# pairlab/leibnizgym

Measured on AMD Instinct MI355X. Metric: env-steps/sec (whole node), trifinger_difficulty_4 @65536 envs, 1/2/4/8 GPUs, higher is better.
Workload: dtype f32

## Files before the change

### leibnizgym_amd/csrc/tf_roles.h

```cpp
#pragma once
#include <type_traits>

#include "tf_contact.h"

#define NT 256

enum { M_ACT_IN = 1, M_RESETS = 2, M_TORQUE = 4, M_SIM = 8, M_POST = 16, M_FINISH = 32, M_ACT_RAND = 64  };
#define M_FUSED_STEP (M_ACT_IN | M_RESETS | M_TORQUE | M_SIM | M_POST | M_FINISH)
#define M_FUSED_STEP_RAND (M_FUSED_STEP | M_ACT_RAND)
#define M_FUSED_RESET (M_RESETS | M_TORQUE | M_SIM | M_POST)

#define L_REC(f) (30 * (f))
#define R_A 0
#define R_DIR 6
#define R_RXD 15
#define R_U 24
#define R_DL 27
#define P_AW 0
#define P_BW 3
#define P_MINV 6
#define P_S1 12
#define P_C1 13
#define P_P2 14
#define P_P3 17
#define P_VQ 20
#define L_POSE_A 23
#define L_POSE_B 53
#define L_WALL 90
#define L_PARK(f) L_REC(f)
#define PK_FC 0
#define PK_LINK 4
#define PK_TF 5
#define PK_TW 8
#define PK_TAU 11
#define PK_FT 14
#define L_VQFF 138
#define L_INIT 147
#define L_DR0 32
#define LDS_SLOTS 159
DEV constexpr int ffm_mbox(int fd, int k, bool boxw = false) {
    return boxw ? 180 + 6 * fd + k
         : fd == 0 ? (k == 0 ? 147 : 149 + k)
         : fd == 1 ? (k == 0 ? 148 : (k == 1 ? 59 : 153 + k))
                   : 83 + k;
}
#define NT_HELP 512
#define L_HELP_OWN 159
#define L_HELP_DR 177
#define LDS_SLOTS_HELP 180
DEV constexpr int ffm_own_mbox(int fm, int k) { return L_HELP_OWN + 6 * fm + k; }
#define L_POSE_S 150
#define LDS_SLOTS_BOX 159
#define LDS_SLOTS_BOX_WIDE 198
#define L_CONE 180
#define LDS_SLOTS_SURF 268
#define L_XCH (MAX_STATES)
#define L_NAN (MAX_STATES + 18)
#define L_VSQ (MAX_STATES + 22)
#define L_OTERM (MAX_STATES + 31)
static_assert(MAX_STATES + 37 <= LDS_SLOTS, "post-phase LDS map");
#define LD(slot) lds[(slot) * WAVE + lane]

struct Ctx {
    int tid, lane, role;
    int wave_first, i, n_valid;
    bool valid;
};

#define ST_RSRC() __builtin_amdgcn_make_buffer_rsrc((void*)P.state, 0, TF_STATE_ROWS * P.N * 4, 0x00020000)
#define LDST(row) __builtin_bit_cast(float, __builtin_amdgcn_raw_buffer_load_b32(ST_RSRC(), (unsigned)cx.i * 4u, (row) * P.N * 4, 0))
#define STST(row, val) do { if (cx.valid) __builtin_amdgcn_raw_buffer_store_b32(__builtin_bit_cast(unsigned, (float)(val)), ST_RSRC(), (unsigned)cx.i * 4u, (row) * P.N * 4, 0); } while (0)
#define BAR() __syncthreads()
#define IN_FLIGHT3(a, b, c) asm volatile("" : "+v"(a), "+v"(b), "+v"(c))
#define IN_FLIGHT4(a, b, c, d) asm volatile("" : "+v"(a), "+v"(b), "+v"(c), "+v"(d))

#ifdef TF_PHASE_TIMING
#define TF_SCR_STRIDE 256
#define NOW() ((uint32_t)__builtin_readcyclecounter())
#define STAMP(id) do { if (cx.lane == 0) ((gu32*)P.scratch)[((size_t)blockIdx.x * 4 + cx.role) * 64 + (id)] = NOW(); } while (0)
#define STAMPV(id, val) do { if (cx.lane == 0) ((gu32*)P.scratch)[((size_t)blockIdx.x * 4 + cx.role) * 64 + (id)] = (uint32_t)(val); } while (0)
#else
#define TF_SCR_STRIDE 16
#define NOW() 0u
#define STAMP(id) do { } while (0)
#define STAMPV(id, val) do { } while (0)
#endif

#define NT_F 192
template <int W, int NTH = NT>
DEV void coop_store_tile(gfloat* __restrict__ dst, const float* lds, const Ctx& cx) {
    const unsigned total = (unsigned)(cx.n_valid * W);
    gfloat* base = dst + (size_t)cx.wave_first * (size_t)W;
    const unsigned total4 = total >> 2;
    const __amdgpu_buffer_rsrc_t tile = __builtin_amdgcn_make_buffer_rsrc((void*)base, 0, (int)(total4 * 16u), 0x00020000);
    constexpr int ITER = (16 * W + NTH - 1) / NTH;
    const unsigned last4 = total4 - 1u;
#pragma unroll
    for (int k = 0; k < ITER; ++k) {
        const unsigned idx = (unsigned)cx.tid + (unsigned)(NTH * k);
        const unsigned src = (idx < last4) ? idx : last4;
        u32x4 vv = *reinterpret_cast<const u32x4*>(&lds[src * 4u]);
        __builtin_amdgcn_raw_buffer_store_b128(vv, tile, idx * 16u, 0, 0);
    }
    const unsigned tail = (total4 << 2) + (unsigned)cx.tid;
    if (tail < total) base[tail] = lds[tail];
}
template <int W, int LS, int NTH = NT>
DEV void coop_store_tile_strided(gfloat* __restrict__ dst, const float* lds, const Ctx& cx) {
    const unsigned total = (unsigned)(cx.n_valid * W);
    gfloat* base = dst + (size_t)cx.wave_first * (size_t)W;
    const unsigned total4 = total >> 2;
    const __amdgpu_buffer_rsrc_t tile = __builtin_amdgcn_make_buffer_rsrc((void*)base, 0, (int)(total4 * 16u), 0x00020000);
    constexpr int ITER = (16 * W + NTH - 1) / NTH;
    const unsigned lastf = total - 1u;
#pragma unroll
    for (int k = 0; k < ITER; ++k) {
        const unsigned idx = (unsigned)cx.tid + (unsigned)(NTH * k);
        u32x4 vv;
#pragma unroll
        for (int e = 0; e < 4; ++e) {
            unsigned g = idx * 4u + (unsigned)e;
            g = (g < lastf) ? g : lastf;
            const unsigned row = g / (unsigned)W, col = g - row * (unsigned)W;
            vv[e] = __builtin_bit_cast(unsigned, lds[row * (unsigned)LS + col]);
        }
        __builtin_amdgcn_raw_buffer_store_b128(vv, tile, idx * 16u, 0, 0);
    }
    const unsigned tail = (total4 << 2) + (unsigned)cx.tid;
    if (tail < total) { const unsigned row = tail / (unsigned)W, col = tail - row * (unsigned)W; base[tail] = lds[row * (unsigned)LS + col]; }
}
template <int A>
DEV void coop_load_tile(const float* __restrict__ src, float* lds, const Ctx& cx) {
    const float* base = src + (size_t)cx.wave_first * (size_t)A;
    const unsigned last = (unsigned)(cx.n_valid * A) - 1u;
    constexpr int ITER = (WAVE * A + NT - 1) / NT;
    float t[ITER];
#pragma unroll
    for (int k = 0; k < ITER; ++k) {
        const unsigned idx = (unsigned)cx.tid + (unsigned)(NT * k);
        t[k] = base[idx < last ? idx : last];
    }
#pragma unroll
    for (int k = 0; k < ITER; ++k) {
        const unsigned idx = (unsigned)cx.tid + (unsigned)(NT * k);
        if (idx < (unsigned)(WAVE * A)) lds[idx] = t[k];
    }
}

template <int A>
DEV void draw_action_tile(const DevParams& P, const StepArgs& sa, float* lds, const Ctx& cx) {
    constexpr int NB = (A + 3) / 4;
    for (int t = cx.tid; t < WAVE * NB; t += NT) {
        const int e = t / NB, b = t - e * NB;
        const int ge = cx.wave_first + ((e < cx.n_valid) ? e : (cx.n_valid - 1));
        float u[4];
        rng4(P, (uint32_t)(P.env_id_offset + ge), sa.frame0, RNG_ACTION + (uint32_t)b, u);
#pragma unroll
        for (int k = 0; k < 4; ++k) {
            const int c = 4 * b + k;
            if (c < A) lds[e * A + c] = 2.0f * u[k] - 1.0f;
        }
    }
}

DEV void sample_xy(float u_r, float u_t, float r_max, float& x, float& y) {
    float radius = f_sqrt(u_r) * r_max;
    float s, c;
    tf_sincos(6.2831855f * u_t, s, c);
    x = radius * c;
    y = radius * s;
}
DEV void sample_yaw_quat(float u, float q[4]) {
    float s, c;
    tf_sincos((6.2831855f * u) * 0.5f, s, c);
    q[0] = 0.0f; q[1] = 0.0f; q[2] = s; q[3] = c;
}
DEV void normalize_quat(const float n[4], float q[4]) {
    float nrm = f_sqrt(n[0] * n[0] + n[1] * n[1] + n[2] * n[2] + n[3] * n[3]);
    float inv = 1.0f / f_max(nrm, 1e-12f);
#pragma unroll
    for (int i = 0; i < 4; ++i) q[i] = n[i] * inv;
}

DEV void sample_goal_pos(const DevParams& P, uint32_t gid, uint32_t count, float xyz[3], float quat[4]) {
    const int d = P.task_difficulty;
    float u[4];
    rng4(P, gid, count, RNG_GOAL_POS, u);
    float x = 0.0f, y = 0.0f, z;
    quat[0] = 0.0f; quat[1] = 0.0f; quat[2] = 0.0f; quat[3] = 1.0f;
    if (d == -1 || d == 1 || d == 3 || d == 4 || d == 5) sample_xy(u[0], u[1], P.m.obj_max_com_dist, x, y);
    if (d == -1 || d == 1) z = P.m.obj_min_height;
// ... 1413 lines not shown
            for (int j = 0; j < 10; ++j) nx_goal[j] = LDST(TF_S_NEXT_GOAL + j);
        }
        const bool draw_now = __builtin_amdgcn_ballot_w64(rflag && !have) != 0ull;
        if (rflag) {
            if (DR && P.dr_enable) draw_dr<EXT>(P, gid, count, dr);
            if (P.object_reset_type == TF_RESET_DEFAULT) {
                cp[0] = EXT ? 0.0f + dr[TF_DR_STAGE_POS] : 0.0f; cp[1] = EXT ? 0.0f + dr[TF_DR_STAGE_POS + 1] : 0.0f; cp[2] = m.obj_min_height * dr[1];
                cq[0] = 0.0f; cq[1] = 0.0f; cq[2] = 0.0f; cq[3] = 1.0f;
#pragma unroll
                for (int k = 0; k < 3; ++k) { cv[k] = 0.0f; cw[k] = 0.0f; }
            } else if (P.object_reset_type == TF_RESET_RANDOM) {
                float ox = nx_obj[0], oy = nx_obj[1], oq[4] = {0.0f, 0.0f, nx_obj[2], nx_obj[3]};
                if (draw_now) {
                    float u[4], tx, ty, tq[4];
                    rng4(P, gid, count, RNG_OBJECT, u);
                    sample_xy(u[0], u[1], m.obj_max_com_dist, tx, ty);
                    sample_yaw_quat(u[2], tq);
                    ox = have ? ox : tx; oy = have ? oy : ty; oq[2] = have ? oq[2] : tq[2]; oq[3] = have ? oq[3] : tq[3];
                }
                cp[0] = EXT ? ox + dr[TF_DR_STAGE_POS] : ox; cp[1] = EXT ? oy + dr[TF_DR_STAGE_POS + 1] : oy;
                cp[2] = m.obj_min_height * dr[1];
#pragma unroll
                for (int k = 0; k < 4; ++k) cq[k] = oq[k];
#pragma unroll
                for (int k = 0; k < 3; ++k) { cv[k] = 0.0f; cw[k] = 0.0f; }
            }
            if (draw_now) {
                float raw[10];
                sample_goal_pos(P, gid, count, &raw[0], &raw[3]);
                sample_goal_rot(P, gid, count, &raw[3], &raw[7]);
#pragma unroll
                for (int j = 0; j < 10; ++j) nx_goal[j] = have ? nx_goal[j] : raw[j];
            }
            goal_from_raw<EXT>(nx_goal, dr, gp, gq, gw);
            count = count + 1u;
#pragma unroll
            for (int j = 0; j < 12; ++j) { lam_cf[j] = 0.0f; lam_cw[j] = 0.0f; }
            cf_face = 0.0f; cw_face = 0.0f;
            n_resets = cx.valid ? 1.0f : 0.0f;
        }
        if (gflag) {
            sample_goal<EXT>(P, gid, count, dr, gp, gq, gw);
            count = count + 1u;
        }
        if (cx.valid) {
            if (rflag) { P.reset_buf[(unsigned)cx.i] = 0; P.steps[(unsigned)cx.i] = 0; P.successes[(unsigned)cx.i] = 0; }
            if (gflag) P.goal_reset_buf[(unsigned)cx.i] = 0;
            if (rflag || gflag) P.reset_count[(unsigned)cx.i] = count;
        }
        if (DR && rflag && P.dr_enable) {
#pragma unroll
            for (int j = 0; j < NDR; ++j) STST(TF_S_DR + j, dr[j]);
        }
        if (rflag || gflag) {
#pragma unroll
            for (int j = 0; j < 3; ++j) { STST(TF_S_GOAL_P + j, gp[j]); STST(TF_S_GOAL_W + j, gw[j]); }
#pragma unroll
            for (int j = 0; j < 4; ++j) STST(TF_S_GOAL_Q + j, gq[j]);
        }
        c_reset = false;
        c_goal_reset = IS_RESET ? (fl_goal_reset != 0) : false;
        c_successes = rflag ? false : (fl_successes != 0);
        c_steps = rflag ? 0 : fl_steps;
    }
    if (MODE & (M_ACT_IN | M_RESETS)) {
        BAR();
        BAR();
        coop_store_tile<A>(P.action_buf, lds, cx);
    }
    if (MODE & M_TORQUE) {
#pragma unroll
        for (int j = 0; j < 3; ++j) STST(TF_S_PREV_OBJ_P + j, cp[j]);
#pragma unroll
        for (int j = 0; j < 4; ++j) STST(TF_S_PREV_OBJ_Q + j, cq[j]);
    }
    STAMP(2);
    if (MODE & M_SIM) {
        const float h = P.hsub, inv_h = 1.0f / h;
        const int nsub = sa.nsim * P.substeps;
        __builtin_amdgcn_s_setprio(3);
#pragma unroll
        for (int c = 0; c < 4; ++c) {
#pragma unroll
            for (int d = 0; d < 3; ++d) LD(L_WALL + 12 * c + 9 + d) = lam_cw[3 * c + d];
        }
        for (int s = 0; s < nsub; ++s) {
            const int sb_ = 4 + 12 * (s & 1);
            (void)sb_;
            float drs[TF_NUM_DR];
#pragma unroll
            for (int j = 0; j < TF_NUM_DR; ++j) drs[j] = (!DR || WIDE || j >= NDR || s == 0 || !P.dr_enable) ? dr[j] : LDST(TF_S_DR + j);
            const float* dr = drs;
            const float cube_mass = m.cube_mass * dr[0];
            const float cube_inertia = m.cube_inertia * dr[0] * dr[1] * dr[1];
            const float inv_m = 1.0f / cube_mass, inv_I = 1.0f / cube_inertia;
            const float fr1 = dr[TF_DR_FRICTION_ROBOT] - 1.0f, fo1 = dr[TF_DR_FRICTION_OBJECT] - 1.0f, fs1 = dr[TF_DR_FRICTION_STAGE] - 1.0f;
            const float mu_fc = (m.mu_finger_cube * dr[2]) * (EXT ? pair_factor(m.mu_robot, fr1, m.mu_object, fo1) : 1.0f);
            const float mu_cf = (m.mu_cube_floor * dr[2]) * (EXT ? pair_factor(m.mu_object, fo1, m.mu_floor, fs1) : 1.0f);
            const float mu_cw = (m.mu_cube_wall * dr[2]) * (EXT ? pair_factor(m.mu_object, fo1, m.mu_stage, fs1) : 1.0f);
            const float soff[2] = {dr[TF_DR_STAGE_POS], dr[TF_DR_STAGE_POS + 1]};
            const float rest_ff = m.restitution_ff * dr[5];
            const float ws = m.warm_start;
            constexpr bool box = BOXK;
            float hc[3];
#pragma unroll
            for (int j = 0; j < 3; ++j) hc[j] = (box ? m.box_half[j] : m.cube_half) * dr[1];
            float v[3], w[3];
            float R[9];
            quat_to_rot(cq, R);
            {
                float wf[3] = {cw[0], cw[1], cw[2]};
                if (__builtin_expect(box && m.box_gyroscopic, 0)) {
                    float wb[3], Iw[3], tq[3];
                    mat3T_mul(R, wf, wb);
#pragma unroll
                    for (int k = 0; k < 3; ++k) Iw[k] = m.box_inertia[k] * wb[k];
                    cross3(Iw, wb, tq);
#pragma unroll
                    for (int k = 0; k < 3; ++k) wb[k] = FMA(h, tq[k] / m.box_inertia[k], wb[k]);
                    mat3_mul(R, wb, wf);
                }
                float dl = 1.0f - h * m.cube_linear_damping, da = 1.0f - h * m.cube_angular_damping;
#pragma unroll
                for (int j = 0; j < 3; ++j) {
                    v[j] = FMA(h, P.grav[j], cv[j]) * dl;
                    w[j] = wf[j] * da;
                }
                if (__builtin_expect(box, 0)) {
                    float sc[3], si[3], S[6], Sinv[6], wh[3];
#pragma unroll
                    for (int k = 0; k < 3; ++k) { sc[k] = f_sqrt(m.cube_inertia / m.box_inertia[k]); si[k] = 1.0f / sc[k]; }
                    rot_diag_rot(R, sc, S);
                    rot_diag_rot(R, si, Sinv);
                    sym3_mul(Sinv, w, wh);
#pragma unroll
                    for (int j = 0; j < 3; ++j) w[j] = wh[j];
#pragma unroll
                    for (int e = 0; e < 6; ++e) LD(L_POSE_S + e) = S[e];
                }
            }
#pragma unroll
            for (int j = 0; j < 3; ++j) { LD(L_POSE_A + j) = cp[j]; LD(L_POSE_B + j) = v[j]; LD(L_POSE_B + 3 + j) = w[j]; }
#pragma unroll
            for (int j = 0; j < 4; ++j) LD(L_POSE_A + 3 + j) = cq[j];
            float fr_[12], fDinv[12], fbias[4], flam[12];
            if constexpr (!WIDE) {
#include "tf_floor_corners.inc"
            }
            bool wall_lane = false;
            bool slot_any[4] = {false, false, false, false};
            unsigned cone_any = 0u;
            constexpr bool WREG = WIDE && !BOXK;
            float w_r[6], w_n[4], w_D[6], w_bias[2], w_lam[6], w_a[6], w_b[6];
            if constexpr (!HELP) {
#include "tf_wall_corners.inc"
            }
            STAMP(sb_ + 0);
            BAR();
            STAMP(sb_ + 1);
            if constexpr (HELP) {
#include "tf_wall_corners.inc"
            } else {
#include "tf_ff_distal.inc"
            }
            if (!WIDE && m.ff_middle_pairs != 0) {
                const TfLinkShape& sh = m.shape2;
                const float jx = m.j3_origin[0], jy = m.j3_origin[1], jz = m.j3_origin[2];
                const float inv_j = f_rcp(FMA(jy, jy, jz * jz));
#pragma unroll 1
                for (int o_ = 2; o_ >= (BOXK ? 1 : 2); --o_)
#pragma unroll 1
                for (int fm = 0; fm < 3; ++fm) {
                    FingerPubRegs pm;
                    read_pub(lds, lane, fm, pm);
                    const Yaw ym = {m.base_yaw_cos[fm], m.base_yaw_sin[fm], 0.0f, 0.0f, m.base_height};
                    const float ex[3] = {pm.k.c1, 0.0f, -pm.k.s1};
                    float ey[3], aw[3], bw[3];
                    {
                        float g[3], xg[3], ez[3], ab[3], bb[3];
#pragma unroll
                        for (int i = 0; i < 3; ++i) g[i] = FMA(-jx, ex[i], pm.k.p3[i] - pm.k.p2[i]);
                        cross3(ex, g, xg);
#pragma unroll
                        for (int i = 0; i < 3; ++i) { ey[i] = FMA(jy, g[i], -(jz * xg[i])) * inv_j; ez[i] = FMA(jz, g[i], jy * xg[i]) * inv_j; }
#pragma unroll
                        for (int i = 0; i < 3; ++i) {
                            ab[i] = FMA(sh.a[2], ez[i], FMA(sh.a[1], ey[i], FMA(sh.a[0], ex[i], pm.k.p2[i])));
                            bb[i] = FMA(sh.b[2], ez[i], FMA(sh.b[1], ey[i], FMA(sh.b[0], ex[i], pm.k.p2[i])));
                        }
                        base_to_world(ym, ab, aw);
                        base_to_world(ym, bb, bw);
                    }
                    {
                        const int o = o_;
                        const int fd = (fm + o >= 3) ? fm + o - 3 : fm + o;
                        float Pm[3], Pd[3], sp;
                        {
                            float Ad[3], Bd[3];
#pragma unroll
                            for (int j = 0; j < 3; ++j) { Ad[j] = LD(L_REC(fd) + P_AW + j); Bd[j] = LD(L_REC(fd) + P_BW + j); }
                            seg_seg_s(aw, bw, Ad, Bd, Pm, Pd, sp);
                        }
                        const float dv[3] = {Pd[0] - Pm[0], Pd[1] - Pm[1], Pd[2] - Pm[2]};
                        const float dist2 = dot3(dv, dv);
                        const float inv = f_rsqrt(f_max(dist2, 1e-12f));
                        const float dist = dist2 * inv;
                        const float n[3] = {dv[0] * inv, dv[1] * inv, dv[2] * inv};
                        float nm[3];
                        dir_world_to_base(ym, n, nm);
                        const float u1 = dot3(nm, ex), u2 = dot3(nm, ey);
                        const float rho = FMA(sp, sh.rho[1] - sh.rho[0], sh.rho[0]);
                        const float h1 = FMA(sp, sh.w1[1] - sh.w1[0], sh.w1[0]) - rho, h2 = FMA(sp, sh.w2[1] - sh.w2[0], sh.w2[0]) - rho;
                        const float o1 = FMA(sp, sh.o1[1] - sh.o1[0], sh.o1[0]), o2 = FMA(sp, sh.o2[1] - sh.o2[0], sh.o2[0]);
                        const float ext = FMA(o2, u2, FMA(o1, u1, FMA(h2, f_abs(u2), FMA(h1, f_abs(u1), rho))));
                        const float gap = dist - ext - m.cap_radius;
                        if ((dist2 > 1e-12f) && (gap < m.contact_margin)) {
                            float Jd[3], Wd[3], Jm[3], Wm[3], vd[3], vm[3];
                            {
                                const Yaw yd = {m.base_yaw_cos[fd], m.base_yaw_sin[fd], 0.0f, 0.0f, m.base_height};
                                FingerPubRegs pd;
                                read_pub(lds, lane, fd, pd);
                                float C[3], Cb_[3], L1[3], L2[3], L3[3], nb[3];
#pragma unroll
                                for (int j = 0; j < 3; ++j) C[j] = FMA(-m.cap_radius, n[j], Pd[j]);
                                world_to_base(yd, C, Cb_);
                                levers(pd.k, Cb_, L1, L2, L3);
                                dir_world_to_base(yd, n, nb);
                                Jd[0] = dot3(L1, nb); Jd[1] = dot3(L2, nb); Jd[2] = dot3(L3, nb);
                                sym3_mul(pd.k.Minv, Jd, Wd);
                            }
                            {
                                float C[3], Cb_[3], L1[3], L2[3], L3[3];
#pragma unroll
                                for (int j = 0; j < 3; ++j) C[j] = FMA(ext, n[j], Pm[j]);
                                world_to_base(ym, C, Cb_);
                                levers(pm.k, Cb_, L1, L2, L3);
                                Jm[0] = dot3(L1, nm); Jm[1] = dot3(L2, nm); Jm[2] = 0.0f;
                                sym3_mul(pm.k.Minv, Jm, Wm);
                            }
#pragma unroll
                            for (int j = 0; j < 3; ++j) { vd[j] = LD(L_REC(fd) + P_VQ + j); vm[j] = LD(L_REC(fm) + P_VQ + j); }
                            const float vn0 = dot3(Jd, vd) - dot3(Jm, vm);
                            if (contact_live(m, gap, vn0, h)) {
                                const float bias = contact_bias(m, gap, vn0, inv_h, rest_ff);
                                const float lam = f_max(-(vn0 + bias) * f_rcp2(dot3(Jd, Wd) + dot3(Jm, Wm)), 0.0f);
#pragma unroll
                                for (int j = 0; j < 3; ++j) {
                                    const float dd = Wd[j] * lam, dm = Wm[j] * lam;
                                    if (dd != 0.0f) LD(L_VQFF + 3 * fd + j) = LD(L_VQFF + 3 * fd + j) + dd;
                                    if (dm != 0.0f) LD(L_VQFF + 3 * fm + j) = LD(L_VQFF + 3 * fm + j) - dm;
                                }
                            }
                        }
                    }
                }
            }
            STAMP(sb_ + 2);
            BAR();
            STAMP(sb_ + 3);
            if constexpr (WIDE) {
#include "tf_floor_corners.inc"
            }
            STAMP(sb_ + 4);
            BAR();
            STAMP(sb_ + 5);
            if constexpr (WIDE && !BOXK) {
            Twist tw;
#pragma unroll
            for (int j = 0; j < 3; ++j) { tw.p[j].x = v[j]; tw.p[j].y = w[j]; }
            float2v mI; mI.x = inv_m; mI.y = inv_I;
            float cDinv[9], cbias[3], clam[9], Km[9];
            float2v rec[27];
#pragma unroll
            for (int f = 0; f < 3; ++f) {
                const int rb = L_REC(f);
                cbias[f] = LD(L_INIT + f);
#pragma unroll
                for (int d = 0; d < 3; ++d) { cDinv[3 * f + d] = LD(L_VQFF + 3 * f + d); clam[3 * f + d] = LD(rb + R_DL + d); Km[3 * f + d] = LD(rb + R_A + d); }
#pragma unroll
                for (int j = 0; j < 9; ++j) { rec[9 * f + j].x = LD(rb + R_DIR + j); rec[9 * f + j].y = LD(rb + R_RXD + j); }
                if (cDinv[3 * f] > 0.0f) {
#pragma unroll
                    for (int d = 0; d < 3; ++d) pk_row_apply_neg(&rec[9 * f + 3 * d], clam[3 * f + d], mI, tw);
                }
            }
#pragma unroll
            for (int c = 0; c < 4; ++c) {
                if (fDinv[3 * c] > 0.0f) {
                    cz_apply(&fr_[3 * c], flam[3 * c], mI, tw);
                    cx_apply(&fr_[3 * c], flam[3 * c + 1], mI, tw);
                    cy_apply(&fr_[3 * c], flam[3 * c + 2], mI, tw);
                }
            }
#pragma unroll
            for (int c = 0; c < 4; ++c) {
                const int wb = L_WALL + 12 * c;
                if (c < 2) {
                    if (slot_any[c] && w_D[3 * c] > 0.0f) {
                        wn_apply(&w_n[2 * c], &w_a[3 * c], w_lam[3 * c], mI, tw);
                        wt_apply(&w_n[2 * c], &w_b[3 * c], w_lam[3 * c + 1], mI, tw);
                        cz_apply(&w_r[3 * c], w_lam[3 * c + 2], mI, tw);
                    }
                } else if (slot_any[c] && LD(wb + 5) > 0.0f) {
                    float r[3] = {LD(wb), LD(wb + 1), LD(wb + 2)}, n[2] = {LD(wb + 3), LD(wb + 4)};
                    float a[3], b[3];
                    wall_arm_n(r, n, a);
                    wall_arm_t(r, n, b);
                    wn_apply(n, a, LD(wb + 9), mI, tw);
// ... 4 lines not shown
            if constexpr (SURF) {
                if (__builtin_expect(cone_any != 0u, 0)) {
#pragma unroll 1
                    for (int c = 0; c < 4; ++c) {
                        const int cb = L_CONE + 22 * c, wb = L_WALL + 12 * c;
                        if (((cone_any >> c) & 1u) && LD(cb + 18) > 0.0f) {
#pragma unroll 1
                            for (int d = 0; d < 3; ++d) pk_row_apply_lds(lds, lane, cb + 6 * d, LD(wb + 9 + d), mI, tw);
                        }
                    }
                }
            }
            uint32_t t_wait = 0u, t_fc = 0u, t_floor = 0u;
            STAMP(sb_ + 9);
            for (int it = 0; it < P.iters; ++it) {
                const uint32_t tf0_ = NOW();
                const bool last = it == P.iters - 1;
                float uu[9];
#pragma unroll
                for (int f = 0; f < 3; ++f) {
#pragma unroll
                    for (int j = 0; j < 3; ++j) uu[3 * f + j] = LD(L_REC(f) + R_U + j);
                }
#pragma unroll
                for (int f = 0; f < 3; ++f) {
#ifdef TF_DIAG_NO_FC
                    if (false) {
#else
                    if (cDinv[3 * f] > 0.0f) {
#endif
                        const int rb = L_REC(f);
                        const float2v* R = &rec[9 * f];
                        float vr[3], dl[3];
                        {
                            float2v p0 = R[0] * tw.p[0], p1 = R[3] * tw.p[0], p2 = R[6] * tw.p[0];
                            p0 = pk_fma(R[1], tw.p[1], p0); p1 = pk_fma(R[4], tw.p[1], p1); p2 = pk_fma(R[7], tw.p[1], p2);
                            p0 = pk_fma(R[2], tw.p[2], p0); p1 = pk_fma(R[5], tw.p[2], p1); p2 = pk_fma(R[8], tw.p[2], p2);
                            vr[0] = uu[3 * f] - (p0.x + p0.y); vr[1] = uu[3 * f + 1] - (p1.x + p1.y); vr[2] = uu[3 * f + 2] - (p2.x + p2.y);
                        }
                        dl[0] = solve_normal(clam[3 * f], cDinv[3 * f], vr[0], cbias[f]);
                        vr[1] = FMA(Km[3 * f], dl[0], vr[1]);
                        dl[1] = solve_tangent(clam[3 * f + 1], cDinv[3 * f + 1], vr[1], mu_fc * clam[3 * f]);
                        vr[2] = FMA(Km[3 * f + 2], dl[1], FMA(Km[3 * f + 1], dl[0], vr[2]));
                        dl[2] = solve_tangent(clam[3 * f + 2], cDinv[3 * f + 2], vr[2], mu_fc * clam[3 * f]);
#pragma unroll
                        for (int d = 0; d < 3; ++d) {
                            LD(rb + R_DL + d) = dl[d];
                            pk_row_apply_neg(&R[3 * d], dl[d], mI, tw);
                        }
                    }
                }
                t_fc += NOW() - tf0_;
                { const uint32_t t0_ = NOW(); BAR(); t_wait += NOW() - t0_; }
#pragma unroll
                for (int c = 0; c < 4; ++c) {
                    const float* r = &fr_[3 * c];
#ifdef TF_DIAG_NO_FLOOR
                    if (false) {
#else
                    if (fDinv[3 * c] > 0.0f) {
#endif
                        float dl = solve_normal(flam[3 * c], fDinv[3 * c], cz_vrel(r, tw), fbias[c]);
                        cz_apply(r, dl, mI, tw);
                        dl = solve_tangent(flam[3 * c + 1], fDinv[3 * c + 1], cx_vrel(r, tw), mu_cf * flam[3 * c]);
                        cx_apply(r, dl, mI, tw);
                        dl = solve_tangent(flam[3 * c + 2], fDinv[3 * c + 2], cy_vrel(r, tw), mu_cf * flam[3 * c]);
                        cy_apply(r, dl, mI, tw);
                    }
                }
                t_floor += NOW() - tf0_;
#pragma unroll
                for (int c = 0; c < 4; ++c) {
#ifdef TF_DIAG_NO_WALL
                    continue;
#endif
                    if (!slot_any[c]) continue;
                    const int wb = L_WALL + 12 * c;
                    if (c < 2) {
                        float dl = solve_normal(w_lam[3 * c], w_D[3 * c], wn_vrel(&w_n[2 * c], &w_a[3 * c], tw), w_bias[c]);
                        wn_apply(&w_n[2 * c], &w_a[3 * c], dl, mI, tw);
                        dl = solve_tangent(w_lam[3 * c + 1], w_D[3 * c + 1], wt_vrel(&w_n[2 * c], &w_b[3 * c], tw), mu_cw * w_lam[3 * c]);
                        wt_apply(&w_n[2 * c], &w_b[3 * c], dl, mI, tw);
                        dl = solve_tangent(w_lam[3 * c + 2], w_D[3 * c + 2], cz_vrel(&w_r[3 * c], tw), mu_cw * w_lam[3 * c]);
                        cz_apply(&w_r[3 * c], dl, mI, tw);
                        if (last && w_D[3 * c] > 0.0f) {
#pragma unroll
                            for (int d = 0; d < 3; ++d) LD(wb + 9 + d) = w_lam[3 * c + d];
                        }
                    } else {
                        float r[3] = {LD(wb), LD(wb + 1), LD(wb + 2)}, n[2] = {LD(wb + 3), LD(wb + 4)};
                        float Dinv[3] = {LD(wb + 5), LD(wb + 6), LD(wb + 7)}, bias = LD(wb + 8);
                        float lam[3] = {LD(wb + 9), LD(wb + 10), LD(wb + 11)};
                        float a[3], b[3];
                        wall_arm_n(r, n, a);
                        wall_arm_t(r, n, b);
                        float dl = solve_normal(lam[0], Dinv[0], wn_vrel(n, a, tw), bias);
                        wn_apply(n, a, dl, mI, tw);
                        dl = solve_tangent(lam[1], Dinv[1], wt_vrel(n, b, tw), mu_cw * lam[0]);
                        wt_apply(n, b, dl, mI, tw);
                        dl = solve_tangent(lam[2], Dinv[2], cz_vrel(r, tw), mu_cw * lam[0]);
                        cz_apply(r, dl, mI, tw);
                        if (Dinv[0] > 0.0f) {
#pragma unroll
                            for (int d = 0; d < 3; ++d) LD(wb + 9 + d) = lam[d];
                        }
                    }
                }
                if constexpr (SURF) {
                    if (__builtin_expect(cone_any != 0u, 0)) {
#pragma unroll
                    for (int c = 0; c < 4; ++c) {
                        const int cb = L_CONE + 22 * c, wb = L_WALL + 12 * c;
                        if (((cone_any >> c) & 1u) && LD(cb + 18) > 0.0f) {
                            float lim = 0.0f;
#pragma unroll
                            for (int d = 0; d < 3; ++d) {
                                const float vr = pk_row_vel_lds(lds, lane, cb + 6 * d, tw);
                                float lam = LD(wb + 9 + d);
                                const float dl = (d == 0) ? solve_normal(lam, LD(cb + 18), vr, LD(cb + 21)) : solve_tangent(lam, LD(cb + 18 + d), vr, lim);
                                lim = (d == 0) ? mu_cw * lam : lim;
                                LD(wb + 9 + d) = lam;
                                pk_row_apply_lds(lds, lane, cb + 6 * d, dl, mI, tw);
                            }
                        }
                    }
                    }
                }
                if (last) {
#pragma unroll
                    for (int f = 0; f < 3; ++f) {
                        const int rb = L_REC(f);
                        float ftv[3] = {0.0f, 0.0f, 0.0f}, Fc[3] = {0.0f, 0.0f, 0.0f};
                        if (cDinv[3 * f] > 0.0f) {
#pragma unroll
                            for (int j = 0; j < 3; ++j) {
                                ftv[j] = FMA(rec[9 * f + 6 + j].x, clam[3 * f + 2], rec[9 * f + 3 + j].x * clam[3 * f + 1]);
                                Fc[j] = FMA(rec[9 * f + j].x, clam[3 * f], ftv[j]) * inv_h;
                            }
                        }
                        LD(L_INIT + f) = clam[3 * f];
#pragma unroll
                        for (int j = 0; j < 3; ++j) { LD(rb + R_A + j) = ftv[j]; LD(rb + R_A + 3 + j) = Fc[j]; }
                    }
                }
                { const uint32_t t0_ = NOW(); BAR(); t_wait += NOW() - t0_; }
            }
            STAMP(sb_ + 6);
            STAMPV(sb_ + 8, t_wait);
            STAMPV(sb_ + 10, t_fc);
            STAMPV(sb_ + 11, t_floor);
#pragma unroll
            for (int j = 0; j < 3; ++j) { v[j] = tw.p[j].x; w[j] = tw.p[j].y; }
            } else {
            float cDinv[9], cbias[3], clam[9];
            constexpr int NRR = WIDE ? 27 : 1, NRA = WIDE ? 9 : 1;
            float rA[NRA], rDir[NRR], rRxd[NRR];
            if (WIDE) {
#pragma unroll
                for (int f = 0; f < 3; ++f) {
#pragma unroll
                    for (int j = 0; j < 3; ++j) rA[(3 * f + j) % NRA] = LD(L_REC(f) + R_A + j);
#pragma unroll
                    for (int j = 0; j < 9; ++j) { rDir[(9 * f + j) % NRR] = LD(L_REC(f) + R_DIR + j); rRxd[(9 * f + j) % NRR] = LD(L_REC(f) + R_RXD + j); }
                }
            }
            int fc_ix[3] = {L_REC(2) * WAVE + lane, L_REC(2) * WAVE + lane, L_REC(2) * WAVE + lane};
#define FC_REC(k, slot) lds[fc_ix[k] + (slot) * WAVE]
            if constexpr (!WIDE) {
                float sD[9], sb[3], sl[9];
#pragma unroll
                for (int f = 0; f < 3; ++f) {
                    sb[f] = LD(L_INIT + f);
#pragma unroll
                    for (int d = 0; d < 3; ++d) { sD[3 * f + d] = LD(L_VQFF + 3 * f + d); sl[3 * f + d] = LD(L_REC(f) + R_DL + d); }
                }
#pragma unroll 1
                for (int f = 0; f < 3; ++f) {
                    const int rb = L_REC(f);
                    if ((f == 0 ? sD[0] : (f == 1 ? sD[3] : sD[6])) > 0.0f) {
#pragma unroll
                        for (int d = 0; d < 3; ++d) {
                            float dir[3], rxd[3];
#pragma unroll
                            for (int j = 0; j < 3; ++j) { dir[j] = LD(rb + R_DIR + 3 * d + j); rxd[j] = LD(rb + R_RXD + 3 * d + j); }
                            const float l = f == 0 ? sl[d] : (f == 1 ? sl[3 + d] : sl[6 + d]);
                            float sc = l * inv_m, qq = l * inv_I;
#pragma unroll
                            for (int j = 0; j < 3; ++j) { v[j] = FMA(-dir[j], sc, v[j]); w[j] = FMA(-rxd[j], qq, w[j]); }
                        }
                    }
                }
                const bool l0 = sD[0] > 0.0f, l1 = sD[3] > 0.0f, l01 = l0 && l1;
                fc_ix[0] = (l0 ? L_REC(0) : (l1 ? L_REC(1) : L_REC(2))) * WAVE + lane;
                fc_ix[1] = (l01 ? L_REC(1) : L_REC(2)) * WAVE + lane;
                cbias[0] = l0 ? sb[0] : (l1 ? sb[1] : sb[2]); cbias[1] = l01 ? sb[1] : sb[2]; cbias[2] = sb[2];
#pragma unroll
                for (int d = 0; d < 3; ++d) {
                    cDinv[d] = l0 ? sD[d] : (l1 ? sD[3 + d] : sD[6 + d]); cDinv[3 + d] = l01 ? sD[3 + d] : sD[6 + d]; cDinv[6 + d] = sD[6 + d];
                    clam[d] = l0 ? sl[d] : (l1 ? sl[3 + d] : sl[6 + d]); clam[3 + d] = l01 ? sl[3 + d] : sl[6 + d]; clam[6 + d] = sl[6 + d];
                }
                cDinv[3] = (l0 || l1) ? cDinv[3] : 0.0f;
                cDinv[6] = l01 ? sD[6] : 0.0f;
                if (cDinv[6] > 0.0f) {
#pragma unroll
                    for (int d = 0; d < 3; ++d) LD(L_REC(2) + R_A + 3 + d) = clam[6 + d];
                }
            } else {
#pragma unroll
                for (int f = 0; f < 3; ++f) {
                    const int rb = L_REC(f);
                    cbias[f] = LD(L_INIT + f);
#pragma unroll
                    for (int d = 0; d < 3; ++d) { cDinv[3 * f + d] = LD(L_VQFF + 3 * f + d); clam[3 * f + d] = LD(rb + R_DL + d); }
                    if (cDinv[3 * f] > 0.0f) {
#pragma unroll
                        for (int d = 0; d < 3; ++d) {
                            const float* dir = &rDir[(9 * f + 3 * d) % NRR];
                            const float* rxd = &rRxd[(9 * f + 3 * d) % NRR];
                            float sc = clam[3 * f + d] * inv_m, qq = clam[3 * f + d] * inv_I;
#pragma unroll
                            for (int j = 0; j < 3; ++j) { v[j] = FMA(-dir[j], sc, v[j]); w[j] = FMA(-rxd[j], qq, w[j]); }
                        }
                    }
                }
            }
#pragma unroll
            for (int c = 0; c < 4; ++c) {
                if (fDinv[3 * c] > 0.0f) {
                    if (__builtin_expect(box, 0)) {
                        float S[6];
#pragma unroll
                        for (int e = 0; e < 6; ++e) S[e] = LD(L_POSE_S + e);
#pragma unroll
                        for (int d = 0; d < 3; ++d) {
                            float n[3], a[3];
                            box_axis(d, n);
                            box_arm(S, &fr_[3 * c], n, a);
                            g_apply(n, a, flam[3 * c + d], inv_m, inv_I, v, w);
                        }
                    } else {
                        cz_apply(&fr_[3 * c], flam[3 * c], inv_m, inv_I, v, w);
                        cx_apply(&fr_[3 * c], flam[3 * c + 1], inv_m, inv_I, v, w);
                        cy_apply(&fr_[3 * c], flam[3 * c + 2], inv_m, inv_I, v, w);
                    }
                }
            }
            {
#pragma unroll
            for (int c = 0; c < 4; ++c) {
                const int wb = L_WALL + 12 * c;
                if (WREG && c < 2) {
                    if (slot_any[c] && w_D[3 * c] > 0.0f) {
                        wn_apply(&w_n[2 * c], &w_a[3 * c], w_lam[3 * c], inv_m, inv_I, v, w);
                        wt_apply(&w_n[2 * c], &w_b[3 * c], w_lam[3 * c + 1], inv_m, inv_I, v, w);
                        cz_apply(&w_r[3 * c], w_lam[3 * c + 2], inv_m, inv_I, v, w);
                    }
                } else
                if (slot_any[c] && LD(wb + 5) > 0.0f) {
                    float r[3] = {LD(wb), LD(wb + 1), LD(wb + 2)}, n[2] = {LD(wb + 3), LD(wb + 4)};
                    float a[3], b[3], c3[3];
                    wall_arms(box, lds, lane, r, n, a, b, c3);
                    wn_apply(n, a, LD(wb + 9), inv_m, inv_I, v, w);
                    wt_apply(n, b, LD(wb + 10), inv_m, inv_I, v, w);
                    if (__builtin_expect(box, 0)) { float ez[3]; box_axis(0, ez); g_apply(ez, c3, LD(wb + 11), inv_m, inv_I, v, w); }
                    else cz_apply(r, LD(wb + 11), inv_m, inv_I, v, w);
                }
            }
            }
            uint32_t t_wait = 0u, t_fc = 0u, t_floor = 0u;
            STAMP(sb_ + 9);
            for (int it = 0; it < P.iters; ++it) {
                const uint32_t tf0_ = NOW();
                const bool last = it == P.iters - 1;
                float uu[9];
                if (WIDE) {
#pragma unroll
                    for (int f = 0; f < 3; ++f) {
#pragma unroll
                        for (int j = 0; j < 3; ++j) uu[3 * f + j] = LD(L_REC(f) + R_U + j);
                    }
                }
#pragma unroll
                for (int f = 0; f < 3; ++f) {
                    const int rb = L_REC(f);
                    if (cDinv[3 * f] > 0.0f) {
                        float Km[3], u[3], dirs[9], rxds[9], vr[3], dl[3];
#pragma unroll
                        for (int j = 0; j < 3; ++j) { Km[j] = WIDE ? rA[(3 * f + j) % NRA] : FC_REC(f, R_A + j); u[j] = WIDE ? uu[3 * f + j] : FC_REC(f, R_U + j); }
#pragma unroll
                        for (int j = 0; j < 9; ++j) { dirs[j] = WIDE ? rDir[(9 * f + j) % NRR] : FC_REC(f, R_DIR + j); rxds[j] = WIDE ? rRxd[(9 * f + j) % NRR] : FC_REC(f, R_RXD + j); }
#pragma unroll
                        for (int d = 0; d < 3; ++d) vr[d] = u[d] - (dot3(&dirs[3 * d], v) + dot3(&rxds[3 * d], w));
                        if (!WIDE && f == 2) {
                            cbias[2] = LD(L_INIT + 2);
#pragma unroll
                            for (int d = 0; d < 3; ++d) clam[6 + d] = LD(L_REC(2) + R_A + 3 + d);
                        }
                        dl[0] = solve_normal(clam[3 * f], cDinv[3 * f], vr[0], cbias[f]);
                        vr[1] = FMA(Km[0], dl[0], vr[1]);
                        dl[1] = solve_tangent(clam[3 * f + 1], cDinv[3 * f + 1], vr[1], mu_fc * clam[3 * f]);
                        vr[2] = FMA(Km[2], dl[1], FMA(Km[1], dl[0], vr[2]));
                        dl[2] = solve_tangent(clam[3 * f + 2], cDinv[3 * f + 2], vr[2], mu_fc * clam[3 * f]);
#pragma unroll
                        for (int d = 0; d < 3; ++d) {
                            if constexpr (WIDE) LD(rb + R_DL + d) = dl[d]; else FC_REC(f, R_DL + d) = dl[d];
                            if (!WIDE && f == 2) LD(L_REC(2) + R_A + 3 + d) = clam[6 + d];
                            const float sc = dl[d] * inv_m, qq = dl[d] * inv_I;
#pragma unroll
                            for (int j = 0; j < 3; ++j) { v[j] = FMA(-dirs[3 * d + j], sc, v[j]); w[j] = FMA(-rxds[3 * d + j], qq, w[j]); }
                        }
                    }
                }
                t_fc += NOW() - tf0_;
                { const uint32_t t0_ = NOW(); BAR(); t_wait += NOW() - t0_; }
#pragma unroll
                for (int c = 0; c < 4; ++c) {
                    const float* r = &fr_[3 * c];
                    if (__builtin_expect(box, 0)) {
                        if (fDinv[3 * c] > 0.0f) {
                            float S[6];
#pragma unroll
                            for (int e = 0; e < 6; ++e) S[e] = LD(L_POSE_S + e);
#pragma unroll
                            for (int d = 0; d < 3; ++d) {
                                float n[3], a[3];
                                box_axis(d, n);
                                box_arm(S, r, n, a);
                                const float vrel = g_vrel(n, a, v, w);
                                const float dlb = (d == 0) ? solve_normal(flam[3 * c], fDinv[3 * c], vrel, fbias[c])
                                                           : solve_tangent(flam[3 * c + d], fDinv[3 * c + d], vrel, mu_cf * flam[3 * c]);
                                g_apply(n, a, dlb, inv_m, inv_I, v, w);
                            }
                        }
                    } else
                    if (fDinv[3 * c] > 0.0f) {
                        float dl = solve_normal(flam[3 * c], fDinv[3 * c], cz_vrel(r, v, w), fbias[c]);
                        cz_apply(r, dl, inv_m, inv_I, v, w);
                        dl = solve_tangent(flam[3 * c + 1], fDinv[3 * c + 1], cx_vrel(r, v, w), mu_cf * flam[3 * c]);
                        cx_apply(r, dl, inv_m, inv_I, v, w);
                        dl = solve_tangent(flam[3 * c + 2], fDinv[3 * c + 2], cy_vrel(r, v, w), mu_cf * flam[3 * c]);
                        cy_apply(r, dl, inv_m, inv_I, v, w);
                    }
                }
                t_floor += NOW() - tf0_;
                {
#pragma unroll
                for (int c = 0; c < 4; ++c) {
                    if (!slot_any[c]) continue;
                    const int wb = L_WALL + 12 * c;
                    if (WREG && c < 2) {
                        float dl = solve_normal(w_lam[3 * c], w_D[3 * c], wn_vrel(&w_n[2 * c], &w_a[3 * c], v, w), w_bias[c]);
                        wn_apply(&w_n[2 * c], &w_a[3 * c], dl, inv_m, inv_I, v, w);
                        dl = solve_tangent(w_lam[3 * c + 1], w_D[3 * c + 1], wt_vrel(&w_n[2 * c], &w_b[3 * c], v, w), mu_cw * w_lam[3 * c]);
                        wt_apply(&w_n[2 * c], &w_b[3 * c], dl, inv_m, inv_I, v, w);
                        dl = solve_tangent(w_lam[3 * c + 2], w_D[3 * c + 2], cz_vrel(&w_r[3 * c], v, w), mu_cw * w_lam[3 * c]);
                        cz_apply(&w_r[3 * c], dl, inv_m, inv_I, v, w);
                        if (last && w_D[3 * c] > 0.0f) {
#pragma unroll
                            for (int d = 0; d < 3; ++d) LD(wb + 9 + d) = w_lam[3 * c + d];
                        }
                    } else {
                        float r[3] = {LD(wb), LD(wb + 1), LD(wb + 2)}, n[2] = {LD(wb + 3), LD(wb + 4)};
                        float Dinv[3] = {LD(wb + 5), LD(wb + 6), LD(wb + 7)}, bias = LD(wb + 8);
                        float lam[3] = {LD(wb + 9), LD(wb + 10), LD(wb + 11)};
                        float a[3], b[3], c3[3];
                        wall_arms(box, lds, lane, r, n, a, b, c3);
                        float dl = solve_normal(lam[0], Dinv[0], wn_vrel(n, a, v, w), bias);
                        wn_apply(n, a, dl, inv_m, inv_I, v, w);
                        dl = solve_tangent(lam[1], Dinv[1], wt_vrel(n, b, v, w), mu_cw * lam[0]);
                        wt_apply(n, b, dl, inv_m, inv_I, v, w);
                        if (__builtin_expect(box, 0)) {
                            float ez[3];
                            box_axis(0, ez);
                            dl = solve_tangent(lam[2], Dinv[2], g_vrel(ez, c3, v, w), mu_cw * lam[0]);
                            g_apply(ez, c3, dl, inv_m, inv_I, v, w);
                        } else {
                            dl = solve_tangent(lam[2], Dinv[2], cz_vrel(r, v, w), mu_cw * lam[0]);
                            cz_apply(r, dl, inv_m, inv_I, v, w);
                        }
                        if (Dinv[0] > 0.0f) {
#pragma unroll
                            for (int d = 0; d < 3; ++d) LD(wb + 9 + d) = lam[d];
                        }
                    }
                }
                }
                if (!WIDE && last) {
#pragma unroll
                    for (int k = 0; k < 2; ++k) {
                        if (cDinv[3 * k] > 0.0f) {
#pragma unroll
                            for (int d = 0; d < 3; ++d) FC_REC(k, R_A + 3 + d) = clam[3 * k + d];
                        }
                    }
#pragma unroll
                    for (int f = 0; f < 3; ++f) {
                        const int rb = L_REC(f);
                        float ftv[3] = {0.0f, 0.0f, 0.0f}, Fc[3] = {0.0f, 0.0f, 0.0f};
                        float l0 = LD(rb + R_DL);
                        if (LD(L_VQFF + 3 * f) > 0.0f) {
                            float dirs[9], l[3];
#pragma unroll
                            for (int j = 0; j < 9; ++j) dirs[j] = LD(rb + R_DIR + j);
#pragma unroll
                            for (int d = 0; d < 3; ++d) l[d] = LD(rb + R_A + 3 + d);
#pragma unroll
                            for (int j = 0; j < 3; ++j) {
                                ftv[j] = FMA(dirs[6 + j], l[2], dirs[3 + j] * l[1]);
                                Fc[j] = FMA(dirs[j], l[0], ftv[j]) * inv_h;
                            }
                            l0 = l[0];
                        }
                        LD(L_INIT + f) = l0;
#pragma unroll
                        for (int j = 0; j < 3; ++j) { LD(rb + R_A + j) = ftv[j]; LD(rb + R_A + 3 + j) = Fc[j]; }
                    }
                }
                if constexpr (WIDE) {
                if (last) {
#pragma unroll
                    for (int f = 0; f < 3; ++f) {
                        const int rb = L_REC(f);
                        float ftv[3] = {0.0f, 0.0f, 0.0f}, Fc[3] = {0.0f, 0.0f, 0.0f};
                        if (cDinv[3 * f] > 0.0f) {
                            const float* dirs = &rDir[(9 * f) % NRR];
#pragma unroll
                            for (int j = 0; j < 3; ++j) {
                                ftv[j] = FMA(dirs[6 + j], clam[3 * f + 2], dirs[3 + j] * clam[3 * f + 1]);
                                Fc[j] = FMA(dirs[j], clam[3 * f], ftv[j]) * inv_h;
                            }
                        }
                        LD(L_INIT + f) = clam[3 * f];
#pragma unroll
                        for (int j = 0; j < 3; ++j) { LD(rb + R_A + j) = ftv[j]; LD(rb + R_A + 3 + j) = Fc[j]; }
                    }
                }
                }
                { const uint32_t t0_ = NOW(); BAR(); t_wait += NOW() - t0_; }
            }
            STAMP(sb_ + 6);
            STAMPV(sb_ + 8, t_wait);
            STAMPV(sb_ + 10, t_fc);
            STAMPV(sb_ + 11, t_floor);
#undef FC_REC
            }
#pragma unroll
            for (int j = 0; j < 12; ++j) lam_cf[j] = flam[j];
            if (__builtin_expect(box, 0)) {
                float S[6], ww[3];
#pragma unroll
                for (int e = 0; e < 6; ++e) S[e] = LD(L_POSE_S + e);
                sym3_mul(S, w, ww);
#pragma unroll
                for (int j = 0; j < 3; ++j) w[j] = ww[j];
            }
#pragma unroll
            for (int j = 0; j < 3; ++j) {
                cv[j] = v[j]; cw[j] = w[j];
                cp[j] = FMA(h, v[j], cp[j]);
            }
            quat_integrate(cq, cw, h);
            STAMP(sb_ + 7);
        }
#pragma unroll
        for (int c = 0; c < 4; ++c) {
#pragma unroll
            for (int d = 0; d < 3; ++d) lam_cw[3 * c + d] = LD(L_WALL + 12 * c + 9 + d);
        }
        __builtin_amdgcn_s_setprio(0);
    }
    STAMP(30);
    StatsTicket tk;
    tk.mine = 0ull; tk.old = 0ull;
    if (MODE & (M_POST | M_FINISH)) {
        c_reset = P.reset_buf[(unsigned)cx.i] != 0;
        c_goal_reset = P.goal_reset_buf[(unsigned)cx.i] != 0;
        c_successes = P.successes[(unsigned)cx.i] != 0;
        c_steps = (int)P.steps[(unsigned)cx.i];
    }
    if (MODE & M_POST) {
        float gp[3], gq[4], prev_obj[7];
#pragma unroll
        for (int j = 0; j < 3; ++j) gp[j] = LDST(TF_S_GOAL_P + j);
#pragma unroll
        for (int j = 0; j < 4; ++j) gq[j] = LDST(TF_S_GOAL_Q + j);
#pragma unroll
        for (int j = 0; j < 7; ++j) prev_obj[j] = LDST(TF_S_PREV_OBJ_P + j);
        LaneStats st;
        stats_zero(st);
        st.resets = n_resets;
        {
            float acc = 0.0f;
#pragma unroll
            for (int j = 0; j < 3; ++j) acc = acc + cp[j] * 0.0f + cv[j] * 0.0f + cw[j] * 0.0f;
#pragma unroll
            for (int j = 0; j < 4; ++j) acc = acc + cq[j] * 0.0f;
            LD(L_NAN + 3) = (acc == 0.0f) ? 0.0f : 1.0f;
        }
        float o_dist = 0.0f, o_ang = 0.0f, o_r[4] = {0.0f, 0.0f, 0.0f, 0.0f};
        auto object_terms = [&]() __attribute__((always_inline)) {
            const RewardCoef& rc = sa.rc;
            o_dist = norm3d(cp, gp);
            o_r[0] = rc.c_dist * lgsk(o_dist, 50.0f);
            o_ang = quat_diff_rad(cq, gq);
            o_r[1] = rc.w_rot * (rc.rot_num / (rc.rot_scale * f_abs(o_ang) + rc.rot_scale));
            const float ang_prev = quat_diff_rad(&prev_obj[3], gq);
            o_r[2] = rc.w_rot_delta * (rc.rot_delta_sched * (f_abs(o_ang) - f_abs(ang_prev)));
            o_r[3] = rc.w_move * (o_dist - norm3d(prev_obj, gp));
        };
        if (!IS_RESET) {
            object_terms();
            if (!WIDE) { LD(L_OTERM) = o_dist; LD(L_OTERM + 1) = o_ang; LD(L_OTERM + 2) = o_r[0]; LD(L_OTERM + 3) = o_r[1]; LD(L_OTERM + 4) = o_r[2]; LD(L_OTERM + 5) = o_r[3]; }
        }
        STAMP(31);
        BAR();
        STAMP(32);
        const bool guarded = (LD(L_NAN) + LD(L_NAN + 1) + LD(L_NAN + 2) + LD(L_NAN + 3)) != 0.0f;
        if (__builtin_expect(guarded, 0)) {
            cp[0] = 0.0f; cp[1] = 0.0f; cp[2] = m.obj_min_height;
            cq[0] = 0.0f; cq[1] = 0.0f; cq[2] = 0.0f; cq[3] = 1.0f;
#pragma unroll
            for (int k = 0; k < 3; ++k) { cv[k] = 0.0f; cw[k] = 0.0f; }
            if (cx.valid) P.reset_buf[(unsigned)cx.i] = 1;
            c_reset = true;
            st.nonfinite += cx.valid ? 1.0f : 0.0f;
            if (!IS_RESET) {
                object_terms();
                if (!WIDE) { LD(L_OTERM) = o_dist; LD(L_OTERM + 1) = o_ang; LD(L_OTERM + 2) = o_r[0]; LD(L_OTERM + 3) = o_r[1]; LD(L_OTERM + 4) = o_r[2]; LD(L_OTERM + 5) = o_r[3]; }
            }
        }
        const float co = P.clip_obs;
        const bool nrm = P.normalize_obs != 0;
        float* row = &lds[lane * TW];
#pragma unroll
        for (int j = 0; j < 3; ++j) { row[18 + j] = emit_scaled(cp[j], PLO(j), 0.3f, nrm, co); row[25 + j] = emit_scaled(gp[j], PLO(j), 0.3f, nrm, co); }
#pragma unroll
        for (int j = 0; j < 4; ++j) { row[21 + j] = emit_scaled(cq[j], -1.0f, 1.0f, nrm, co); row[28 + j] = emit_scaled(gq[j], -1.0f, 1.0f, nrm, co); }
        if (ASYM) {
#pragma unroll
            for (int j = 0; j < 3; ++j) { row[OD + j] = emit_scaled(cv[j], -0.5f, 0.5f, nrm, co); row[OD + 3 + j] = emit_scaled(cw[j], -0.5f, 0.5f, nrm, co); }
        }
        auto add_noise = [&]() {
            float nz[28];
#pragma unroll
            for (int b = 4; b < 7; ++b) rng4(P, gid, sa.frame, RNG_OBS_NOISE + (uint32_t)b, &nz[4 * b]);
#pragma unroll
            for (int jj = 18; jj < 25; ++jj) row[jj] = f_clamp(FMA(P.dr_obs_noise, 2.0f * nz[jj] - 1.0f, row[jj]), -co, co);
        };
        if (DR && !ASYM && P.dr_obs_noise > 0.0f) add_noise();
        STAMP(33);
        BAR();
        STAMP(34);
        if (!IS_RESET) {
            float tips[9], tip_prev[9];
#pragma unroll
            for (int f = 0; f < 3; ++f) {
#pragma unroll
                for (int j = 0; j < 3; ++j) { tips[3 * f + j] = LD(L_XCH + 6 * f + j); tip_prev[3 * f + j] = LD(L_XCH + 6 * f + 3 + j); }
            }
            const RewardCoef& rc = sa.rc;
            float r[6];
            {
                float s = 0.0f;
                s = s + (norm_p3(&tips[0], cp, P.norm_p) - norm_p3(&tip_prev[0], prev_obj, P.norm_p));
                s = s + (norm_p3(&tips[3], cp, P.norm_p) - norm_p3(&tip_prev[3], prev_obj, P.norm_p));
                s = s + (norm_p3(&tips[6], cp, P.norm_p) - norm_p3(&tip_prev[6], prev_obj, P.norm_p));
                r[0] = rc.c_reach * s;
            }
            {
                float s = 0.0f;
#pragma unroll
                for (int j = 0; j < 9; ++j) s = s + LD(L_VSQ + j);
                r[1] = rc.c_move_pen * s;
            }
            if (!WIDE) { o_dist = LD(L_OTERM); o_ang = LD(L_OTERM + 1); o_r[0] = LD(L_OTERM + 2); o_r[1] = LD(L_OTERM + 3); o_r[2] = LD(L_OTERM + 4); o_r[3] = LD(L_OTERM + 5); }
            const float dist = o_dist, ang = o_ang;
            r[2] = o_r[0]; r[3] = o_r[1]; r[4] = o_r[2]; r[5] = o_r[3];
            float total = 0.0f;
#pragma unroll
            for (int t = 0; t < 6; ++t) {
                r[t] = guarded ? 0.0f : r[t];
                if (P.rew_active[t]) { total = total + r[t]; st.rew[t] += cx.valid ? r[t] : 0.0f; }
            }
            bool pos_ok = dist <= P.pos_tol;
            bool ori_ok = ang <= P.ori_tol;
            st.pos_cnt += (cx.valid && pos_ok) ? 1.0f : 0.0f;
            st.ori_cnt += (cx.valid && ori_ok) ? 1.0f : 0.0f;
            bool done;
            if (P.task_difficulty < 4) done = pos_ok;
            else if (P.task_difficulty == 4) done = pos_ok && ori_ok;
            else done = ori_ok;
            bool succ = c_successes;
            if (P.success_activate) {
                if (done) total = total + P.success_bonus;
                if (cx.valid) P.goal_reset_buf[(unsigned)cx.i] = (uint8_t)done;
                c_goal_reset = done;
// ... 63 lines not shown
```

Before: 1.017 billion.

## Keep wall slot 0 in registers, spill pose to LDS, and loop other wall slots

For the narrow, non-box contact path, wall contact slot 0's arm geometry is held in registers. Slots 1-3 are handled in a non-unrolled loop gated by a bitmask. The cube pose (cp, cq, cw_face) is parked in LDS during the solver loop and restored afterwards, which frees registers. The aim is to lower register pressure and code size in the PGS iteration loop. It also adds extra timing stamps for wall, hand and wait phases, which cost some instructions.

```diff
diff --git a/leibnizgym_amd/csrc/tf_roles.h b/leibnizgym_amd/csrc/tf_roles.h
--- a/leibnizgym_amd/csrc/tf_roles.h
+++ b/leibnizgym_amd/csrc/tf_roles.h
@@ -37,6 +37,7 @@
 #define L_VQFF 138
 #define L_INIT 147
 #define L_DR0 32
+#define L_CPARK 150
 #define LDS_SLOTS 159
 DEV constexpr int ffm_mbox(int fd, int k, bool boxw = false) {
     return boxw ? 180 + 6 * fd + k
@@ -1756,8 +1757,10 @@
             unsigned cone_any = 0u;
             constexpr bool WREG = WIDE && !BOXK;
             float w_r[6], w_n[4], w_D[6], w_bias[2], w_lam[6], w_a[6], w_b[6];
+            unsigned slot_mask = 0u;
             if constexpr (!HELP) {
 #include "tf_wall_corners.inc"
+                slot_mask = (slot_any[0] ? 1u : 0u) | (slot_any[1] ? 2u : 0u) | (slot_any[2] ? 4u : 0u) | (slot_any[3] ? 8u : 0u);
             }
             STAMP(sb_ + 0);
             BAR();
@@ -2068,6 +2071,14 @@
 #pragma unroll
             for (int j = 0; j < 3; ++j) { v[j] = tw.p[j].x; w[j] = tw.p[j].y; }
             } else {
+            constexpr bool CPARK = !WIDE && !BOXK;
+            if constexpr (CPARK) {
+#pragma unroll
+                for (int j = 0; j < 3; ++j) LD(L_CPARK + j) = cp[j];
+#pragma unroll
+                for (int j = 0; j < 4; ++j) LD(L_CPARK + 3 + j) = cq[j];
+                LD(L_CPARK + 7) = cw_face;
+            }
             float cDinv[9], cbias[3], clam[9];
             constexpr int NRR = WIDE ? 27 : 1, NRA = WIDE ? 9 : 1;
             float rA[NRA], rDir[NRR], rRxd[NRR];
@@ -2161,6 +2172,8 @@
                     }
                 }
             }
+            constexpr bool W0REG = !WIDE && !BOXK;
+            float q_r[3] = {0.0f, 0.0f, 0.0f}, q_n[2] = {0.0f, 0.0f};
             {
 #pragma unroll
             for (int c = 0; c < 4; ++c) {
@@ -2171,6 +2184,20 @@
                         wt_apply(&w_n[2 * c], &w_b[3 * c], w_lam[3 * c + 1], inv_m, inv_I, v, w);
                         cz_apply(&w_r[3 * c], w_lam[3 * c + 2], inv_m, inv_I, v, w);
                     }
+                } else
+                if (W0REG && c == 0) {
+#pragma unroll
+                    for (int j = 0; j < 3; ++j) q_r[j] = LD(wb + j);
+                    q_n[0] = LD(wb + 3); q_n[1] = LD(wb + 4);
+                    if ((slot_mask & 1u) != 0u && LD(wb + 5) > 0.0f) {
+                        float a[3], b[3], c3[3];
+                        wall_arms(box, lds, lane, q_r, q_n, a, b, c3);
+                        wn_apply(q_n, a, LD(wb + 9), inv_m, inv_I, v, w);
+                        wt_apply(q_n, b, LD(wb + 10), inv_m, inv_I, v, w);
+                        cz_apply(q_r, LD(wb + 11), inv_m, inv_I, v, w);
+                    }
+                } else
+                if (W0REG) {
                 } else
                 if (slot_any[c] && LD(wb + 5) > 0.0f) {
                     float r[3] = {LD(wb), LD(wb + 1), LD(wb + 2)}, n[2] = {LD(wb + 3), LD(wb + 4)};
@@ -2183,7 +2210,22 @@
                 }
             }
             }
-            uint32_t t_wait = 0u, t_fc = 0u, t_floor = 0u;
+            if (W0REG && (slot_mask & 14u) != 0u) {
+#pragma unroll 1
+                for (int c = 1; c < 4; ++c) {
+                    const int wb = L_WALL + 12 * c;
+                    if (((slot_mask >> c) & 1u) && LD(wb + 5) > 0.0f) {
+                        float r[3] = {LD(wb), LD(wb + 1), LD(wb + 2)}, n[2] = {LD(wb + 3), LD(wb + 4)};
+                        float a[3], b[3];
+                        wall_arm_n(r, n, a);
+                        wall_arm_t(r, n, b);
+                        wn_apply(n, a, LD(wb + 9), inv_m, inv_I, v, w);
+                        wt_apply(n, b, LD(wb + 10), inv_m, inv_I, v, w);
+                        cz_apply(r, LD(wb + 11), inv_m, inv_I, v, w);
+                    }
+                }
+            }
+            uint32_t t_wait = 0u, t_fc = 0u, t_floor = 0u, t_wall = 0u, t_hand = 0u, t_w2 = 0u, n_blk = 0u;
             STAMP(sb_ + 9);
             for (int it = 0; it < P.iters; ++it) {
                 const uint32_t tf0_ = NOW();
@@ -2229,6 +2271,12 @@
                 }
                 t_fc += NOW() - tf0_;
                 { const uint32_t t0_ = NOW(); BAR(); t_wait += NOW() - t0_; }
+                float q_D[3] = {0.0f, 0.0f, 0.0f}, q_bias = 0.0f, q_lam[3] = {0.0f, 0.0f, 0.0f};
+                if (W0REG) {
+#pragma unroll
+                    for (int j = 0; j < 3; ++j) { q_D[j] = LD(L_WALL + 5 + j); q_lam[j] = LD(L_WALL + 9 + j); }
+                    q_bias = LD(L_WALL + 8);
+                }
 #pragma unroll
                 for (int c = 0; c < 4; ++c) {
                     const float* r = &fr_[3 * c];
@@ -2259,10 +2307,13 @@
                     }
                 }
                 t_floor += NOW() - tf0_;
+                const uint32_t tw0_ = NOW();
+                n_blk += (slot_any[0] ? 1u : 0u) + (slot_any[1] ? 1u : 0u) + (slot_any[2] ? 1u : 0u) + (slot_any[3] ? 1u : 0u);
                 {
 #pragma unroll
                 for (int c = 0; c < 4; ++c) {
-                    if (!slot_any[c]) continue;
+                    if (W0REG && c > 0) continue;
+                    if (W0REG ? (slot_mask & 1u) == 0u : !slot_any[c]) continue;
                     const int wb = L_WALL + 12 * c;
                     if (WREG && c < 2) {
                         float dl = solve_normal(w_lam[3 * c], w_D[3 * c], wn_vrel(&w_n[2 * c], &w_a[3 * c], v, w), w_bias[c]);
@@ -2274,6 +2325,19 @@
                         if (last && w_D[3 * c] > 0.0f) {
 #pragma unroll
                             for (int d = 0; d < 3; ++d) LD(wb + 9 + d) = w_lam[3 * c + d];
+                        }
+                    } else if (W0REG && c == 0) {
+                        float a[3], b[3], c3[3];
+                        wall_arms(box, lds, lane, q_r, q_n, a, b, c3);
+                        float dl = solve_normal(q_lam[0], q_D[0], wn_vrel(q_n, a, v, w), q_bias);
+                        wn_apply(q_n, a, dl, inv_m, inv_I, v, w);
+                        dl = solve_tangent(q_lam[1], q_D[1], wt_vrel(q_n, b, v, w), mu_cw * q_lam[0]);
+                        wt_apply(q_n, b, dl, inv_m, inv_I, v, w);
+                        dl = solve_tangent(q_lam[2], q_D[2], cz_vrel(q_r, v, w), mu_cw * q_lam[0]);
+                        cz_apply(q_r, dl, inv_m, inv_I, v, w);
+                        if (q_D[0] > 0.0f) {
+#pragma unroll
+                            for (int d = 0; d < 3; ++d) LD(wb + 9 + d) = q_lam[d];
                         }
                     } else {
                         float r[3] = {LD(wb), LD(wb + 1), LD(wb + 2)}, n[2] = {LD(wb + 3), LD(wb + 4)};
@@ -2301,6 +2365,31 @@
                     }
                 }
                 }
+                if (W0REG && (slot_mask & 14u) != 0u) {
+#pragma unroll 1
+                    for (int c = 1; c < 4; ++c) {
+                        if (!((slot_mask >> c) & 1u)) continue;
+                        const int wb = L_WALL + 12 * c;
+                        float r[3] = {LD(wb), LD(wb + 1), LD(wb + 2)}, n[2] = {LD(wb + 3), LD(wb + 4)};
+                        float Dinv[3] = {LD(wb + 5), LD(wb + 6), LD(wb + 7)}, bias = LD(wb + 8);
+                        float lam[3] = {LD(wb + 9), LD(wb + 10), LD(wb + 11)};
+                        float a[3], b[3];
+                        wall_arm_n(r, n, a);
+                        wall_arm_t(r, n, b);
+                        float dl = solve_normal(lam[0], Dinv[0], wn_vrel(n, a, v, w), bias);
+                        wn_apply(n, a, dl, inv_m, inv_I, v, w);
+                        dl = solve_tangent(lam[1], Dinv[1], wt_vrel(n, b, v, w), mu_cw * lam[0]);
+                        wt_apply(n, b, dl, inv_m, inv_I, v, w);
+                        dl = solve_tangent(lam[2], Dinv[2], cz_vrel(r, v, w), mu_cw * lam[0]);
+                        cz_apply(r, dl, inv_m, inv_I, v, w);
+                        if (Dinv[0] > 0.0f) {
+#pragma unroll
+                            for (int d = 0; d < 3; ++d) LD(wb + 9 + d) = lam[d];
+                        }
+                    }
+                }
+                const uint32_t th0_ = NOW();
+                t_wall += th0_ - tw0_;
                 if (!WIDE && last) {
 #pragma unroll
                     for (int k = 0; k < 2; ++k) {
@@ -2352,12 +2441,23 @@
                     }
                 }
                 }
-                { const uint32_t t0_ = NOW(); BAR(); t_wait += NOW() - t0_; }
+                { const uint32_t t0_ = NOW(); t_hand += t0_ - th0_; BAR(); const uint32_t t1_ = NOW(); t_wait += t1_ - t0_; t_w2 += t1_ - t0_; }
+            }
+            if constexpr (CPARK) {
+#pragma unroll
+                for (int j = 0; j < 3; ++j) cp[j] = LD(L_CPARK + j);
+#pragma unroll
+                for (int j = 0; j < 4; ++j) cq[j] = LD(L_CPARK + 3 + j);
+                cw_face = LD(L_CPARK + 7);
             }
             STAMP(sb_ + 6);
             STAMPV(sb_ + 8, t_wait);
             STAMPV(sb_ + 10, t_fc);
             STAMPV(sb_ + 11, t_floor);
+            STAMPV(40 + 4 * (s & 1), n_blk);
+            STAMPV(41 + 4 * (s & 1), t_wall);
+            STAMPV(42 + 4 * (s & 1), t_hand);
+            STAMPV(43 + 4 * (s & 1), t_w2);
 #undef FC_REC
             }
 #pragma unroll
```

Result: no change. 1.008 billion (-0.9%).
